# kan-bayashi/espnet

Measured on AMD Instinct MI355X. Metric: frames/sec, 12L Conformer hybrid CTC/attention training step (B=32 T=1000 d=256 per GPU), higher is better.
Workload: dtype f32; 1 GPU; BASELINE configs[1]: 12L Conformer enc d=256 h=4 ff=2048 k=31 macaron+cnn rel_pos, 6L Transformer dec, V=5000, fbank B=32 T=1000 L=100, mtlalpha 0.3, lsm 0.1; global_batch=32, frames=1000, parallelism=dp1, optimizer=adam+noam, clip 5.0, launch=hipGraph, wgrad_side_stream=False, optimizer_steps_done=113

## Files before the change

espnet_amd/csrc/gemm.hip:

```cpp
#include <stdlib.h>
#include "common.h"
#include "../../include/espnet_amd.h"

namespace {

constexpr int BK = 32;
constexpr int NTHREADS = 256;

template <int BM, int BN, int PREC>
struct Smem {
  static constexpr int LDK = PREC ? 40 : 36;
  using elem_t = typename std::conditional<PREC == 1, unsigned short, float>::type;
  elem_t a[2][BM][LDK];
  elem_t b[2][BN][LDK];
  int poff[3][BK];
};

struct RowState {
  int base;
  int ih, jw;
  int ok;
};

__device__ __forceinline__ RowState decompose(const eamd_gather_t& g, int row, int nrows) {
  RowState s;
  s.ok = row < nrows;
  int r = s.ok ? row : 0;
  int j = r % g.Wo;
  int t = r / g.Wo;
  int i = t % g.Ho;
  int b = t / g.Ho;
  s.base = b * g.Hin * g.Win;
  s.ih = i * g.sh;
  s.jw = j * g.sw;
  return s;
}

__device__ __forceinline__ long gather_off(const eamd_gather_t& g, const RowState& s, int tap) {
  int hh = s.ih + g.dh[tap];
  int ww = s.jw + g.dw[tap];
  bool ok = s.ok && hh >= 0 && hh < g.Hin && ww >= 0 && ww < g.Win;
  return ok ? ((long)(s.base + hh * g.Win + ww)) * g.C : -1L;
}

__device__ __forceinline__ float4 apply_act4(float4 v, int act) {
  if (act == EAMD_ACT_SWISH) {
    v.x = eamd_swish(v.x); v.y = eamd_swish(v.y); v.z = eamd_swish(v.z); v.w = eamd_swish(v.w);
  } else if (act == EAMD_ACT_RELU) {
    v.x = fmaxf(v.x, 0.f); v.y = fmaxf(v.y, 0.f); v.z = fmaxf(v.z, 0.f); v.w = fmaxf(v.w, 0.f);
  }
  return v;
}

__device__ __forceinline__ float4 load_kcontig(const float* __restrict__ rowp, bool row_ok, int k, int K,
                                               bool vec_ok) {
  float4 v = make_float4(0.f, 0.f, 0.f, 0.f);
  if (row_ok) {
    if (vec_ok && k + 3 < K) {
      v = *reinterpret_cast<const float4*>(rowp + k);
    } else {
      if (k + 0 < K) v.x = rowp[k + 0];
      if (k + 1 < K) v.y = rowp[k + 1];
      if (k + 2 < K) v.z = rowp[k + 2];
      if (k + 3 < K) v.w = rowp[k + 3];
    }
  }
  return v;
}

__device__ __forceinline__ float4 load_kstrided(const float* __restrict__ p, long ld, bool col_ok, int k,
                                                int K) {
  float4 v = make_float4(0.f, 0.f, 0.f, 0.f);
  if (col_ok) {
    const float* q = p + (long)k * ld;
    if (k + 3 < K) {
      v.x = q[0]; v.y = q[ld]; v.z = q[2 * ld]; v.w = q[3 * ld];
    } else {
      if (k + 0 < K) v.x = q[0];
      if (k + 1 < K) v.y = q[ld];
      if (k + 2 < K) v.z = q[2 * ld];
      if (k + 3 < K) v.w = q[3 * ld];
    }
  }
// ... 301 lines not shown
      if (p.precision == 0 && tile == 128 && t128 > 256 && t128 < 400 && p.splitk == 1) tile = 64;
    }
  }
  if (tile != 64 && tile != 128) return EAMD_EINVAL;

  if (p.gather.enabled) {
    const eamd_gather_t& g = p.gather;
    if (g.ntap < 1 || g.ntap > 9 || g.C <= 0 || g.C % BK != 0) return EAMD_EINVAL;
    if (!p.transA) {
      if (p.K != g.ntap * g.C) return EAMD_EINVAL;
    } else {
      if (p.M != g.ntap * g.C) return EAMD_EINVAL;
      if (g.C % tile != 0) return EAMD_EINVAL;
    }
  }
  if ((p.N + tile - 1) / tile > 65535) return EAMD_EUNSUPPORTED;
  if (p.h_dtype != 0 && p.h_dtype != 1) return EAMD_EINVAL;
  if (p.in_dtype == 1 && p.h_dtype != 0) return EAMD_EUNSUPPORTED;
  if (p.in_dtype != 1 && ((p.Hb && !(p.h_dtype == 1 && p.precision == 0)) || (p.drop_p != 0.f && p.precision != 0)))
    return EAMD_EUNSUPPORTED;
  if ((p.a_drop_p != 0.f || p.b_drop_p != 0.f) && (p.in_dtype != 0 || p.precision != 0)) return EAMD_EUNSUPPORTED;
  tile_out = tile;
  return EAMD_OK;
}

extern "C" int eamd_gemm(const eamd_gemm_t* pp, void* stream_) {
  if (!pp) return EAMD_EINVAL;
  eamd_gemm_t p = *pp;
  hipStream_t stream = (hipStream_t)stream_;
  int tile = 0;
  const int chk = gemm_check(p, tile);
  if (chk != EAMD_OK) return chk;
  const bool stats = p.epilogue == 7, rowgrad = p.epilogue == 8;
  if (p.in_dtype == 1) return eamd_gemm_bf16_dispatch(p, tile, stream);

  if (p.precision == 1 && p.gather.enabled && p.transA && !p.Hb && p.drop_p == 0.f && p.a_drop_p == 0.f &&
      p.b_drop_p == 0.f) {
    const int rc = eamd_gemm_f32_dispatch(p, tile, stream);
    if (rc != EAMD_EUNSUPPORTED) return rc;
  }
  if (p.precision == 0) {
    const int rc = eamd_gemm_f32_dispatch(p, tile, stream);
    if (rc != EAMD_EUNSUPPORTED) return rc;
    if (p.drop_p != 0.f || p.a_drop_p != 0.f || p.b_drop_p != 0.f || p.Hb) return EAMD_EUNSUPPORTED;
  }
  if (stats || rowgrad) return EAMD_EUNSUPPORTED;
  if (tile == 128) {
    return p.precision ? launch<128, 128, 1>(p, stream) : launch<128, 128, 0>(p, stream);
  }
  return p.precision ? launch<64, 64, 1>(p, stream) : launch<64, 64, 0>(p, stream);
}

int eamd_gemm_f32_multi(const eamd_gemm_t* ps, const int* tiles, int n, hipStream_t stream);

extern "C" int eamd_gemm_multi(const eamd_gemm_t* descs, int n, void* stream) {
  if (!descs || n < 1) return EAMD_EINVAL;
  if (n >= 2 && n <= EAMD_GEMM_MULTI_MAX) {
    eamd_gemm_t ps[EAMD_GEMM_MULTI_MAX];
    int tiles[EAMD_GEMM_MULTI_MAX];
    bool f32 = true;
    for (int i = 0; i < n; ++i) {
      ps[i] = descs[i];
      const int chk = gemm_check(ps[i], tiles[i]);
      if (chk != EAMD_OK) return chk;
      f32 = f32 && ps[i].in_dtype == 0 && ps[i].precision == 0;
    }
    if (f32) {
      const int rc = eamd_gemm_f32_multi(ps, tiles, n, (hipStream_t)stream);
      if (rc != EAMD_EUNSUPPORTED) return rc;
    }
  }
  for (int i = 0; i < n; ++i) {
    const int rc = eamd_gemm(&descs[i], stream);
    if (rc != EAMD_OK) return rc;
  }
  return EAMD_OK;
}

int eamd_gemm_f32_group_count(const eamd_gemm_t& p);
int eamd_gemm_f32_group_launch(const eamd_gemm_t* tab, const int* first, int n, int total, int tile, hipStream_t s);
int eamd_gemm_bf16_group_count(const eamd_gemm_t& p);
int eamd_gemm_bf16_group_launch(const eamd_gemm_t* tab, const int* first, int n, int total, int tile, hipStream_t s);

extern "C" int eamd_gemm_group_plan(const eamd_gemm_t* descs, int n, int32_t* first) {
  if (!descs || !first || n <= 0) return EAMD_EINVAL;
  long total = 0;
  for (int i = 0; i < n; ++i) {
    const eamd_gemm_t& p = descs[i];
    if (!p.A || !p.B || !p.C || p.M <= 0 || p.N <= 0 || p.K <= 0) return EAMD_EINVAL;
    if (p.in_dtype != descs[0].in_dtype || p.precision != descs[0].precision) return EAMD_EINVAL;
    if ((p.tile == 128) != (descs[0].tile == 128)) return EAMD_EINVAL;
    const int c = p.in_dtype == 1 ? eamd_gemm_bf16_group_count(p) : eamd_gemm_f32_group_count(p);
    if (c < 0) return c;
    first[i] = (int32_t)total;
    total += c;
    if (total >= (1L << 30)) return EAMD_EUNSUPPORTED;
  }
  first[n] = (int32_t)total;
  return (int)total;
}

extern "C" int eamd_gemm_group_launch(const eamd_gemm_t* descs_dev, const int32_t* first_dev, int n, int total, int in_dtype,
                                      int tile, void* stream) {
  if (!descs_dev || !first_dev || n <= 0 || total <= 0 || (tile != 64 && tile != 128)) return EAMD_EINVAL;
  return in_dtype == 1 ? eamd_gemm_bf16_group_launch(descs_dev, first_dev, n, total, tile, (hipStream_t)stream)
                       : eamd_gemm_f32_group_launch(descs_dev, first_dev, n, total, tile, (hipStream_t)stream);
}

extern "C" int eamd_abi_version(void) { return 1; }
```

espnet_amd/csrc/gemm_bf16.hip:

```cpp
#include <stdlib.h>
#include <type_traits>
#include "common.h"
#include "../../include/espnet_amd.h"

#include "gemm_bf16_common.h"

namespace {

template <int BM, int BN, bool TA, bool TB, bool FAST, bool GAT, bool ACT, bool ROWEPI = false>
__device__ __forceinline__ void gemm_bf16_body(const eamd_gemm_t& p, const int bid, const int nblk, const int zb) {
  constexpr int WM = BM / 2, WN = BN / 2;
  constexpr int MT = WM / 16, NTL = WN / 16;
  constexpr int NCA = BM / 32, NCB = BN / 32;
  constexpr int CPR_A = BM / 8, RPP_A = NT_ / CPR_A;
  constexpr int CPR_B = BN / 8, RPP_B = NT_ / CPR_B;
  using S = SmemB<BM, BN, TA, TB>;
  extern __shared__ __attribute__((aligned(16))) char smem_raw[];
  S& sm = *reinterpret_cast<S*>(smem_raw);

  const int t = threadIdx.x;
  const int lane = t & 63, wave = t >> 6;
  const int wm = wave >> 1, wn = wave & 1;
  const int tiles_n = (p.N + BN - 1) / BN;
  int tile_id, split;
  if (nblk < 0) {
    const int ntile = ((p.M + BM - 1) / BM) * tiles_n;
    const int per = (-nblk) >> 3;
    const int v = (bid & 7) * per + (bid >> 3);
    if (v >= ntile * p.splitk) return;
    split = v / ntile;
    tile_id = v - split * ntile;
  } else if (p.splitk > 1) {
    split = bid % p.splitk;
    tile_id = bid / p.splitk;
  } else {
    split = 0;
    const int ntile = nblk;
    const int id = bid, q = ntile >> 3, r = ntile & 7, xcd = id & 7, j = id >> 3;
    tile_id = (xcd < r ? xcd * (q + 1) : r * (q + 1) + (xcd - r) * q) + j;
  }
  const int tile_m = tile_id / tiles_n, tile_n = tile_id % tiles_n;
  const int m0 = tile_m * BM, n0 = tile_n * BN;
  const int b1 = zb / p.batch2, b2 = zb % p.batch2;
  const bf16_t* __restrict__ A = reinterpret_cast<const bf16_t*>(p.A) + b1 * p.sA1 + b2 * p.sA2;
  const bf16_t* __restrict__ B = reinterpret_cast<const bf16_t*>(p.B) + b1 * p.sB1 + b2 * p.sB2;
  const long coff = b1 * p.sC1 + b2 * p.sC2;

  const int nkt_total = (p.K + BK - 1) / BK;
  const int per = (nkt_total + p.splitk - 1) / p.splitk;
  const int kt_begin = split * per;
  const int kt_end = min(nkt_total, kt_begin + per);
  const int nkt = kt_end - kt_begin;

  constexpr bool gat = GAT;
  const bool a_vec = (p.lda % 8 == 0) && ((reinterpret_cast<uintptr_t>(A) & 15) == 0);
  const bool b_vec = (p.ldb % 8 == 0) && ((reinterpret_cast<uintptr_t>(B) & 15) == 0);

  int a_r[NCA], a_c[NCA], b_r[NCB], b_c[NCB];
#pragma unroll
  for (int i = 0; i < NCA; ++i) {
    if constexpr (TA) { a_r[i] = t / CPR_A + RPP_A * i; a_c[i] = t % CPR_A; }
    else              { a_r[i] = t / 8 + 32 * i;        a_c[i] = t % 8; }
  }
#pragma unroll
  for (int i = 0; i < NCB; ++i) {
    if constexpr (TB) { b_r[i] = t / CPR_B + RPP_B * i; b_c[i] = t % CPR_B; }
    else              { b_r[i] = t / 8 + 32 * i;        b_c[i] = t % 8; }
  }
  long a_off[NCA], b_off[NCB];
  if constexpr (FAST && !gat) {
#pragma unroll
    for (int i = 0; i < NCA; ++i) {
      if constexpr (!TA) a_off[i] = (long)min(m0 + a_r[i], p.M - 1) * p.lda + a_c[i] * 8;
      else a_off[i] = (long)a_r[i] * p.lda + min(m0 + a_c[i] * 8, (p.M - 1) & ~7);
    }
  }
  if constexpr (FAST) {
#pragma unroll
    for (int i = 0; i < NCB; ++i) {
      if constexpr (!TB) b_off[i] = (long)min(n0 + b_r[i], p.N - 1) * p.ldb + b_c[i] * 8;
      else b_off[i] = (long)b_r[i] * p.ldb + min(n0 + b_c[i] * 8, (p.N - 1) & ~7);
    }
  }
  RowStateB a_rs[NCA];
  if constexpr (gat && !TA) {
#pragma unroll
    for (int i = 0; i < NCA; ++i) a_rs[i] = decompose_b(p.gather, m0 + a_r[i], p.M);
  }
  GatherRegs gr = {0ull, 0ull, 1, 0, 0};
  if constexpr (gat) gr = gather_regs(p.gather);
  constexpr int DEPTH = BM >= 128 ? 3 : 4;
  constexpr int UNROLL = DEPTH % 2 ? 2 * DEPTH : DEPTH;
  uint4 ra[DEPTH][NCA], rb[DEPTH][NCB];
  const bool do_colsum = TA && p.colsum != nullptr && !gat && tile_n == 0;
  float cs[8];
#pragma unroll
  for (int j = 0; j < 8; ++j) cs[j] = 0.f;

  auto fill_poff = [&](int kt, int slot) __attribute__((always_inline)) {
    if (t < BK) {
      const int tap = m0 / gr.C;
      RowStateB s = decompose_b(p.gather, kt * BK + t, p.K);
      sm.poff[slot][t] = (int)gather_off_r(gr, s, tap);
    }
  };

  auto load_tile = [&](auto set_c, auto guard_c, int kt) __attribute__((always_inline)) {
    constexpr int SET = decltype(set_c)::value;
    constexpr bool GUARD = decltype(guard_c)::value;
    const int k0 = kt * BK;
    if constexpr (!TA) {
      if constexpr (!gat) {
#pragma unroll
        for (int i = 0; i < NCA; ++i) {
          const int m = m0 + a_r[i], k = k0 + a_c[i] * 8;
          if constexpr (FAST) {
            const int kk = (GUARD && k >= p.K) ? -a_c[i] * 8 : k0;
            ra[SET][i] = *reinterpret_cast<const uint4*>(A + a_off[i] + kk);
          } else {
            const int nv = m < p.M ? min(8, p.K - k) : 0;
            ra[SET][i] = load8(A, (long)m * p.lda + k, nv, a_vec);
          }
        }
      } else {
        const int tap = k0 / gr.C, c0 = k0 - tap * gr.C;
#pragma unroll
        for (int i = 0; i < NCA; ++i) {
          const long off = gather_off_r(gr, a_rs[i], tap);
          ra[SET][i] = load8_fast(A, off + c0 + a_c[i] * 8, off >= 0 ? 8 : 0);
        }
      }
    } else {
      if constexpr (!gat) {
#pragma unroll
// ... 416 lines not shown
```

espnet_amd/csrc/gemm_f32.hip:

```cpp
#include <stdlib.h>
#include <type_traits>
#include "common.h"
#include "../../include/espnet_amd.h"

#include "gemm_bf16_common.h"

namespace {

constexpr int FBK = 32;

template <int BM, int BN, bool TA, bool TB>
struct SmemF {
  static constexpr int KPAD_A = BM >= 128 ? 8 : 4, KPAD_B = BN >= 128 ? 8 : 4;
  static constexpr int LDA = TA ? BM + KPAD_A : FBK + 4;
  static constexpr int RA = TA ? FBK : BM;
  static constexpr int LDB = TB ? BN + KPAD_B : FBK + 4;
  static constexpr int RB = TB ? FBK : BN;
  static constexpr int OPS = 2 * (RA * LDA + RB * LDB);
  static constexpr int CT = BM * (BN + 4);
  float ab[OPS > CT ? OPS : CT];
  int poff[8][FBK];
  __device__ float* a(int buf) { return ab + buf * RA * LDA; }
  __device__ float* b(int buf) { return ab + 2 * RA * LDA + buf * RB * LDB; }
};

__device__ __forceinline__ float4 act4(float4 v, int act) {
  if (act == EAMD_ACT_SWISH) return make_float4(eamd_swish(v.x), eamd_swish(v.y), eamd_swish(v.z), eamd_swish(v.w));
  return make_float4(fmaxf(v.x, 0.f), fmaxf(v.y, 0.f), fmaxf(v.z, 0.f), fmaxf(v.w, 0.f));
}
__device__ __forceinline__ float4 mask4(float4 v, int nv) {
  return make_float4(nv > 0 ? v.x : 0.f, nv > 1 ? v.y : 0.f, nv > 2 ? v.z : 0.f, nv > 3 ? v.w : 0.f);
}

template <int BM, int BN, bool TA, bool TB, bool GAT, bool ACT, bool ROWEPI = false, bool NOPAD = false>
__device__ __forceinline__ void gemm_f32_body(const eamd_gemm_t& p, const int bid, const int nblk, const int zb) {
  constexpr int WM = BM / 2, WN = BN / 2;
  constexpr int MT = WM / 16, NTL = WN / 16;
  constexpr int NCA = BM / 32, NCB = BN / 32;
  constexpr int CPR_A = BM / 4, RPP_A = NT_ / CPR_A;
  constexpr int CPR_B = BN / 4, RPP_B = NT_ / CPR_B;
  using S = SmemF<BM, BN, TA, TB>;
  extern __shared__ __attribute__((aligned(16))) char smem_raw[];
  S& sm = *reinterpret_cast<S*>(smem_raw);

  const int t = threadIdx.x;
  const int lane = t & 63, wave = t >> 6;
  const int wm = wave >> 1, wn = wave & 1;
  const int tiles_n = (p.N + BN - 1) / BN;
  int tile_id, split;
  if (nblk < 0) {
    const int ntile = ((p.M + BM - 1) / BM) * tiles_n;
    const int per = (-nblk) >> 3;
    const int v = (bid & 7) * per + (bid >> 3);
    if (v >= ntile * p.splitk) return;
    split = v / ntile;
    tile_id = v - split * ntile;
  } else if (p.splitk > 1) {
    split = bid % p.splitk;
    tile_id = bid / p.splitk;
  } else {
    split = 0;
    const int ntile = nblk;
    const int id = bid, q = ntile >> 3, r = ntile & 7, xcd = id & 7, j = id >> 3;
    tile_id = (xcd < r ? xcd * (q + 1) : r * (q + 1) + (xcd - r) * q) + j;
  }
  const int tile_m = tile_id / tiles_n, tile_n = tile_id % tiles_n;
  const int m0 = tile_m * BM, n0 = tile_n * BN;
  const int b1 = zb / p.batch2, b2 = zb % p.batch2;
  const float* __restrict__ A = p.A + b1 * p.sA1 + b2 * p.sA2;
  const float* __restrict__ B = p.B + b1 * p.sB1 + b2 * p.sB2;
  const long coff = b1 * p.sC1 + b2 * p.sC2;

  const int nkt_total = (p.K + FBK - 1) / FBK;
  const int per = (nkt_total + p.splitk - 1) / p.splitk;
  const int kt_begin = split * per;
  const int kt_end = min(nkt_total, kt_begin + per);
  const int nkt = kt_end - kt_begin;

  int a_r[NCA], a_c[NCA], b_r[NCB], b_c[NCB];
#pragma unroll
  for (int i = 0; i < NCA; ++i) {
    if constexpr (TA) { a_r[i] = t / CPR_A + RPP_A * i; a_c[i] = t % CPR_A; }
    else              { a_r[i] = t / 8 + 32 * i;        a_c[i] = t % 8; }
  }
#pragma unroll
  for (int i = 0; i < NCB; ++i) {
    if constexpr (TB) { b_r[i] = t / CPR_B + RPP_B * i; b_c[i] = t % CPR_B; }
    else              { b_r[i] = t / 8 + 32 * i;        b_c[i] = t % 8; }
  }
  long a_off[NCA], b_off[NCB];
  if constexpr (!GAT) {
#pragma unroll
    for (int i = 0; i < NCA; ++i) {
      if constexpr (!TA) a_off[i] = (long)min(m0 + a_r[i], p.M - 1) * p.lda + a_c[i] * 4;
      else a_off[i] = (long)a_r[i] * p.lda + min(m0 + a_c[i] * 4, (p.M - 1) & ~3);
    }
  }
#pragma unroll
  for (int i = 0; i < NCB; ++i) {
    if constexpr (!TB) b_off[i] = (long)min(n0 + b_r[i], p.N - 1) * p.ldb + b_c[i] * 4;
    else b_off[i] = (long)b_r[i] * p.ldb + min(n0 + b_c[i] * 4, (p.N - 1) & ~3);
  }
  RowStateB a_rs[NCA];
  unsigned long long dh_pack = 0ull, dw_pack = 0ull;
  int gC = 1, gHin = 0, gWin = 0;
  if constexpr (GAT) {
#pragma unroll
    for (int tp = 0; tp < 9; ++tp) {
      dh_pack |= (unsigned long long)((unsigned)(p.gather.dh[tp] + 8) & 15u) << (4 * tp);
      dw_pack |= (unsigned long long)((unsigned)(p.gather.dw[tp] + 8) & 15u) << (4 * tp);
    }
    gC = p.gather.C; gHin = p.gather.Hin; gWin = p.gather.Win;
  }
  const int pK = p.K;
  const long ldaL = p.lda, ldbL = p.ldb;
  auto tap_dh = [&](int tap) __attribute__((always_inline)) { return (int)((dh_pack >> (4 * tap)) & 15ull) - 8; };
  auto tap_dw = [&](int tap) __attribute__((always_inline)) { return (int)((dw_pack >> (4 * tap)) & 15ull) - 8; };
  auto goff = [&](const RowStateB& rs, int dh, int dw) __attribute__((always_inline)) -> long {
    const int hh = rs.ih + dh, ww = rs.jw + dw;
    const bool ok = rs.ok && hh >= 0 && hh < gHin && ww >= 0 && ww < gWin;
    return ok ? ((long)(rs.base + hh * gWin + ww)) * gC : -1L;
  };
  constexpr bool g_nopad = NOPAD;
  if constexpr (GAT && !TA) {
#pragma unroll
    for (int i = 0; i < NCA; ++i) a_rs[i] = decompose_b(p.gather, m0 + a_r[i], p.M);
  }
  int pr_row = 0, pr_j = 0, pr_i = 0, pr_b = 0;
  if constexpr (GAT && TA) {
    if (t < FBK) {
      pr_row = kt_begin * FBK + t;
      pr_j = pr_row % p.gather.Wo;
      const int tt = pr_row / p.gather.Wo;
      pr_i = tt % p.gather.Ho;
      pr_b = tt / p.gather.Ho;
    }
  }
  constexpr int DEPTH = BM >= 128 ? 2 : 3;
  constexpr int UNROLL = DEPTH % 2 ? 2 * DEPTH : DEPTH;
  float4 ra[DEPTH][NCA], rb[DEPTH][NCB];
  const unsigned a_dseed = (ACT && p.a_drop_p > 0.f) ? eamd_drop_seed((const unsigned long long*)p.drop_step, p.a_drop_salt) : 0u;
  const unsigned b_dseed = (ACT && p.b_drop_p > 0.f) ? eamd_drop_seed((const unsigned long long*)p.drop_step, p.b_drop_salt) : 0u;
  const bool do_colsum = TA && p.colsum != nullptr && !GAT && tile_n == 0;
  float cs[4] = {0.f, 0.f, 0.f, 0.f};

  const int gWo = GAT ? p.gather.Wo : 1, gHo = GAT ? p.gather.Ho : 1, gsh = GAT ? p.gather.sh : 0, gsw = GAT ? p.gather.sw : 0;
  const int ta_tap = (GAT && TA) ? m0 / gC : 0;
  const int ta_dh = tap_dh(ta_tap), ta_dw = tap_dw(ta_tap);
  auto fill_poff = [&](int kt, int slot) __attribute__((always_inline)) {
    if (t < FBK) {
      RowStateB s;
      s.ok = pr_row < pK;
      s.base = pr_b * gHin * gWin; s.ih = pr_i * gsh; s.jw = pr_j * gsw;
      sm.poff[slot][t] = (int)goff(s, ta_dh, ta_dw);
      pr_row += FBK; pr_j += FBK;
      while (pr_j >= gWo) { pr_j -= gWo; ++pr_i; }
      while (pr_i >= gHo) { pr_i -= gHo; ++pr_b; }
    }
  };
// ... 523 lines not shown
```

espnet_amd/ops.py:

```python
import ctypes as C
import os
import math

import torch

from . import _lib
from ._lib import GatherT, GemmT, RowMapT, check, ptr, stream_ptr

ACT_NONE, ACT_RELU, ACT_SWISH = 0, 1, 2
EPI_NONE, EPI_RELU, EPI_SWISH, EPI_MUL_RELU_MASK, EPI_MUL_DSWISH, EPI_MUL_AUX, EPI_DACT_FACTOR, EPI_ROW_STATS, EPI_ROW_GRAD = 0, 1, 2, 3, 4, 5, 6, 7, 8

_PRECISIONS = {"fp32": 0, "bf16": 1}
_state = {"precision": 0}


def set_precision(name):
    if name not in _PRECISIONS:
        raise ValueError(f"precision must be one of {list(_PRECISIONS)}")
    _state["precision"] = _PRECISIONS[name]


def get_precision():
    return [k for k, v in _PRECISIONS.items() if v == _state["precision"]][0]

# ... 95 lines not shown
        assert (Cm is None and Cb is None) if epilogue == EPI_ROW_STATS else Cm is not None
    c32 = Cm if (Cm is not None and Cm.dtype == torch.float32) else None
    c16 = Cb if Cb is not None else (Cm if (Cm is not None and Cm.dtype == torch.bfloat16) else None)
    if c16 is not None and (c16.dtype != torch.bfloat16 or not bf):
        raise _lib.EamdError("gemm: bf16 outputs need bf16 operands")
    for tt in (R, bias, colsum):
        if tt is not None and tt.dtype != torch.float32:
            raise _lib.EamdError("gemm: bias / residual / colsum must be float32")
    b1, b2 = batch
    if gather is None:
        a_span = _span(K, lda, M) if transA else _span(M, lda, K)
        a_need = a_off + (b1 - 1) * sA[0] + (b2 - 1) * sA[1] + a_span
        if a_need > A.numel():
            raise _lib.EamdError(f"gemm: A too small ({A.numel()} < {a_need})")
    b_span = _span(K, ldb, N) if transB else _span(N, ldb, K)
    b_need = b_off + (b1 - 1) * sB[0] + (b2 - 1) * sB[1] + b_span
    if b_need > B.numel():
        raise _lib.EamdError(f"gemm: B too small ({B.numel()} < {b_need})")
    if cmap is None:
        c_need = c_off + (b1 - 1) * sC[0] + (b2 - 1) * sC[1] + _span(M, ldc, N)
        for ct in (c32, c16):
            if ct is not None and c_need > ct.numel():
                raise _lib.EamdError(f"gemm: C too small ({ct.numel()} < {c_need})")
    if bias is not None and bias.numel() < N:
        raise _lib.EamdError("gemm: bias too small")

    p = GemmT()
    p.A, p.B = ptr(A, a_off), ptr(B, b_off)
    p.C = ptr(c32, c_off) if c32 is not None else None
    p.Cb = ptr(c16, c_off) if c16 is not None else None
    p.bias = ptr(bias)
    p.aux = ptr(aux, c_off) if aux is not None else None
    p.aux_dtype = 1 if (aux is not None and aux.dtype == torch.bfloat16) else 0
    p.R = ptr(R, c_off) if R is not None else None
    if colsum is not None:
        if not transA or gather is not None or colsum.numel() < M * b1 * b2:
            raise _lib.EamdError("gemm: colsum needs transA, no gather and M outputs")
        p.colsum = ptr(colsum)
    p.M, p.N, p.K = M, N, K
    p.transA, p.transB = int(transA), int(transB)
    p.lda, p.ldb, p.ldc, p.ldaux, p.ldr = lda, ldb, ldc, ldaux or ldc, ldr or ldc
    p.batch1, p.batch2 = b1, b2
    p.sA1, p.sA2 = sA
    p.sB1, p.sB2 = sB
    p.sC1, p.sC2 = sC
    p.alpha, p.beta = alpha, beta
    p.a_act, p.b_act, p.epilogue = a_act, b_act, epilogue
    p.splitk = splitk
    p.in_dtype = 1 if bf else 0
    p.precision = 1 if bf else (_state["precision"] if precision is None else precision)
    p.tile = tile
    if stats is not None and epilogue == EPI_ROW_GRAD:
        rowc, col, fix, gscale, scale = stats
        if rowc.dtype != torch.float32 or rowc.numel() < 3 * M or col.dtype != torch.int32 or col.numel() < M or not (0 <= fix < N):
            raise _lib.EamdError("gemm: row-gradient coefficients too small or of the wrong dtype")
        p.stats.rowc, p.stats.col, p.stats.fix, p.stats.gscale, p.stats.scale = ptr(rowc), ptr(col), int(fix), ptr(gscale), float(scale)
    elif stats is not None:
        part, col, zcol, zfix, fix = stats
        tn = (N + tile - 1) // tile
        if part.dtype != torch.float32 or part.numel() < M * tn * 2 or zfix.numel() < M or not (0 <= fix < N) or \
                (col is not None and (col.dtype != torch.int32 or col.numel() < M or zcol is None or zcol.numel() < M)):
            raise _lib.EamdError("gemm: row-statistics buffers too small or of the wrong dtype")
        p.stats.part, p.stats.col, p.stats.zcol, p.stats.zfix, p.stats.fix = ptr(part), ptr(col), ptr(zcol), ptr(zfix), int(fix)
    if gather is not None:
        p.gather = gather
    if cmap is not None:
        p.cmap = cmap
    if drop is not None and drop[0] > 0.0:
        if ldc != N or c_off != 0 or (not bf and p.precision != 0):
            raise _lib.EamdError("gemm: fused dropout needs a contiguous [M, N] result and bf16 or fp32-MFMA operands")
        p.drop_p, p.drop_salt = float(drop[0]), int(drop[1])
        p.drop_step = ptr(rng_state(A.device))
        if Hb is not None:
            if Hb.dtype != (torch.bfloat16 if bf else torch.float32) or Hb.numel() < M * N:
                raise _lib.EamdError("gemm: Hb must be an [M, N] buffer of the operand dtype")
            p.Hb, p.h_act, p.h_dtype = ptr(Hb), h_act, 0 if bf else 1
    for which, d, ld_, off_, cols in (("a", a_drop, lda, a_off, (M if transA else K)), ("b", b_drop, ldb, b_off, (N if transB else K))):
        if d is not None and d[0] > 0.0:
            if bf or p.precision != 0 or ld_ != cols or off_ != 0 or b1 * b2 != 1 or gather is not None:
                raise _lib.EamdError("gemm: operand dropout needs an fp32-MFMA launch on a dense, unbatched operand")
            setattr(p, which + "_drop_p", float(d[0]))
            setattr(p, which + "_drop_salt", int(d[1]))
            p.drop_step = ptr(rng_state(A.device))
    if group and _wgroup["on"] and _in_grad_arena(Cm) and _wgroup_accepts(p):
        lo = Cm.data_ptr() + 4 * c_off
        hi = lo + 4 * _span(M, ldc, N)
        nbytes = A.numel() * A.element_size() + B.numel() * B.element_size()
        clash = any(lo < qhi and qlo < hi and (splitk == 1 or qsk == 1) for qlo, qhi, qsk in _wgroup["ranges"])
        if clash or _wgroup["bytes"] + nbytes > GROUP_WGRAD_MAX_BYTES:
            wgrad_group_flush()
        _wgroup["items"].append((p, (A, B, Cm, colsum)))
        _wgroup["ranges"].append((lo, hi, splitk))
        _wgroup["bytes"] += nbytes
        return
    if defer is not None:
        defer.append((p, (A, B, Cm, bias, aux, R, colsum, Cb, Hb, stats)))
        return
    if _gemm_record is not None:
        _gemm_record.append((p, (A, B, Cm, bias, aux, R, colsum, Cb, Hb, stats),
                             lambda sp, p=p: check(_lib.lib().eamd_gemm(C.byref(p), sp), "eamd_gemm")))
    check(_lib.lib().eamd_gemm(C.byref(p), stream_ptr()), "eamd_gemm")


GEMM_MULTI_MAX = 4


def gemm_multi(items):
    L = _lib.lib()
    for i0 in range(0, len(items), GEMM_MULTI_MAX):
        part = items[i0:i0 + GEMM_MULTI_MAX]
        arr = (GemmT * len(part))(*[it[0] for it in part])
        n = len(part)
        if _gemm_record is not None and any(it[0].in_dtype != 0 or it[0].precision != 0 for it in part):
            for p_, keep in part:
                _gemm_record.append((p_, keep, lambda sp, p_=p_: check(L.eamd_gemm(C.byref(p_), sp), "eamd_gemm")))
        elif _gemm_record is not None:
            _gemm_record.append((dict(kind="multi%d" % n, flop=sum(2.0 * it[0].M * it[0].N * it[0].K for it in part)),
                                 (arr, [it[1] for it in part]),
                                 lambda sp, arr=arr, n=n: check(L.eamd_gemm_multi(arr, n, sp), "eamd_gemm_multi")))
        check(L.eamd_gemm_multi(arr, n, stream_ptr()), "eamd_gemm_multi")


GROUP_WGRAD = True
STACK_WGRAD_MAX_ROWS = 64
GROUP_WGRAD_MAX_TILES = 384
GROUP_WGRAD_SK_DIV = 2
GROUP_WGRAD_TILE128_MIN = 100
GROUP_WGRAD_T128_WGS = 96
GROUP_WGRAD_MAX_BYTES = 16 << 30
_wgroup = {"on": False, "items": [], "ranges": [], "bytes": 0, "stack": {}, "pinned": [], "reserve": [], "arenas": {}}


def register_grad_arena(t):
    import weakref
    key = t.untyped_storage().data_ptr()
    _wgroup["arenas"][key] = weakref.ref(t)


def _in_grad_arena(t):
    key = t.untyped_storage().data_ptr()
    ref = _wgroup["arenas"].get(key)
    if ref is None:
        return False
    a = ref()
    if a is None or a.untyped_storage().data_ptr() != key:
        del _wgroup["arenas"][key]
        return False
    return True


def wgrad_group_begin():
    _wgroup["on"] = GROUP_WGRAD
    _wgroup["items"], _wgroup["stack"] = [], {}
    _wgroup["ranges"], _wgroup["bytes"] = [], 0


def _wgroup_accepts(p):
    if ((p.M + 63) // 64) * ((p.N + 63) // 64) > GROUP_WGRAD_MAX_TILES:
        return False
    first = (C.c_int32 * 2)()
    return _lib.lib().eamd_gemm_group_plan(C.byref(p), 1, first) > 0


def _wgroup_staging(nbytes):
    if torch.cuda.is_current_stream_capturing():
        for i, h in enumerate(_wgroup["reserve"]):
            if h.numel() >= nbytes:
                _wgroup["pinned"].append(_wgroup["reserve"].pop(i))
                return _wgroup["pinned"][-1][:nbytes]
        return None
    want = (nbytes + 4095) // 4096 * 4096 * 2
    _wgroup["reserve"] = [h for h in _wgroup["reserve"] if h.numel() >= want]
    while len(_wgroup["reserve"]) < 16:
        _wgroup["reserve"].append(torch.empty(want, dtype=torch.uint8, pin_memory=True))
    return torch.empty(nbytes, dtype=torch.uint8, pin_memory=True)


def wgrad_group_flush():
    stack, _wgroup["stack"] = _wgroup["stack"], {}
    for dW, db, dys, xs in stack.values():
        if len(dys) == 1:
            dyc, xc = dys[0], xs[0]
        else:
            dyc, xc = torch.cat(dys, 0), torch.cat(xs, 0)
        if dyc.shape[0] <= STACK_WGRAD_MAX_ROWS:
            sk = auto_splitk(dyc.shape[1], xc.shape[1], dyc.shape[0])
            gemm(dyc, xc, dW, dyc.shape[1], xc.shape[1], dyc.shape[0], dyc.shape[1], xc.shape[1], xc.shape[1], transA=1,
                 transB=1, splitk=sk, beta=1.0 if sk == 1 else 0.0, colsum=db, group=True)
        else:
            _linear_bwd_w(dyc, xc, dW, db=db)
    items = _wgroup["items"]
    if not items:
        return
    _wgroup["items"], _wgroup["ranges"], _wgroup["bytes"] = [], [], 0
    for tile in (64, 128):
        part = [it for it in items if (128 if it[0].tile == 128 else 64) == tile]
        if part:
            _wgroup_launch(part, tile)


def _wgroup_launch(items, tile):
    L = _lib.lib()

    def separately():
        for p, keep in items:
            if _gemm_record is not None:
                _gemm_record.append((p, keep, lambda sp, p=p: check(L.eamd_gemm(C.byref(p), sp), "eamd_gemm")))
            check(L.eamd_gemm(C.byref(p), stream_ptr()), "eamd_gemm")

    if len(items) == 1:
        return separately()
    n = len(items)
    dev = items[0][1][0].device
    arr = (GemmT * n)(*[it[0] for it in items])
    first = (C.c_int32 * (n + 1))()
    total = L.eamd_gemm_group_plan(arr, n, first)
    check(min(total, 0), "eamd_gemm_group_plan")
    nb_desc, nb_first = C.sizeof(arr), C.sizeof(first)
    host = _wgroup_staging(nb_desc + nb_first)
    if host is None:
        return separately()
    C.memmove(host.data_ptr(), arr, nb_desc)
    C.memmove(host.data_ptr() + nb_desc, first, nb_first)
    tab = torch.empty(nb_desc + nb_first, dtype=torch.uint8, device=dev)
    tab.copy_(host, non_blocking=True)
    in_dtype = int(arr[0].in_dtype)
    args = (ptr(tab), ptr(tab, nb_desc), n, total, in_dtype, tile)
    check(L.eamd_gemm_group_launch(*args, stream_ptr()), "eamd_gemm_group_launch")
    if _gemm_record is not None:
        _gemm_record.append((dict(kind="group%d" % tile, flop=sum(2.0 * it[0].M * it[0].N * it[0].K * it[0].batch1 * it[0].batch2 for it in items)),
                             (tab, [it[1] for it in items]),
                             lambda sp, args=args: check(L.eamd_gemm_group_launch(*args, sp), "eamd_gemm_group_launch")))


def cast_bf16(x, out=None):
    if out is None:
        out = torch.empty(x.shape, device=x.device, dtype=torch.bfloat16)
    assert x.dtype == torch.float32 and x.is_contiguous() and out.numel() == x.numel()
    check(_lib.lib().eamd_cast_bf16(ptr(x), ptr(out), C.c_int64(x.numel()), stream_ptr()), "eamd_cast_bf16")
    return out


def auto_splitk(m_out, n_out, k_red):
    tiles = ((m_out + 63) // 64) * ((n_out + 63) // 64)
    if tiles >= 512:
        return 1
    want = 4.0 * (128.0 / tiles) ** 0.5
    s = 1
    while s < want:
        s *= 2
    return max(1, min(s, 64, max(1, k_red // 128)))


LINEAR_ROWS = True
_infer = 0


class inference:

    def __enter__(self):
        global _infer
        _infer += 1

    def __exit__(self, *exc):
        global _infer
        _infer -= 1
        return False


def inference_call(fn):
    import functools

    @functools.wraps(fn)
    def wrapped(*a, **k):
        with inference():
            return fn(*a, **k)
    return wrapped
LINEAR_ROWS_MAX = 16
LINEAR_ROWS_BLOCK_MAX = 1024
LINEAR_ROWS_KSPLIT = True


def linear_fwd(x, W, b, out=None, *, act=EPI_NONE, R=None, alpha=1.0, a_act=ACT_NONE, out_dtype=torch.float32,
               drop=None, Hb=None, h_act=ACT_NONE, a_drop=None):
    M, K = x.shape
    N = W.shape[0]
    assert W.shape[1] == K and W.is_contiguous() and x.stride(1) == 1 and (R is None or R.stride(-1) == 1)
    if (LINEAR_ROWS and (M <= LINEAR_ROWS_MAX or (M <= LINEAR_ROWS_BLOCK_MAX and (K <= 512 or (K >= 1024 and LINEAR_ROWS_KSPLIT)) and N <= 1024
# ... 314 lines not shown
    if out is None:
        out = torch.empty(M, N, device=dev, dtype=torch.float32)
    p = _lib.RowProjT()
    p.a, p.lda, p.w, p.bias = ptr(a), a.stride(0), ptr(img), ptr(bias)
    p.R, p.ldr = ptr(R), (R.stride(0) if R is not None else 0)
    p.out, p.ldo = ptr(out), out.stride(0)
    p.M, p.K, p.N, p.alpha = M, K, N, float(alpha)
    if drop is not None and drop[0] > 0.0:
        p.p_out, p.salt_out, p.drop_step = float(drop[0]), int(drop[1]), ptr(rng_state(dev))
    if ln is not None:
        xr, g, b, eps, mean, rstd = ln
        p.ln_x, p.ln_w, p.ln_b, p.ln_mean, p.ln_rstd, p.ln_eps = ptr(xr), ptr(g), ptr(b), ptr(mean), ptr(rstd), float(eps)
    if affine is not None:
        sc, sh, act, a_out = affine
        p.a_scale, p.a_shift, p.a_act, p.a_out = ptr(sc), ptr(sh), int(act), ptr(a_out)
    if lnb is not None:
        xb, g, mean, rstd, dres, ws, d_out, d_ps = lnb
        p.lnb_x, p.lnb_gamma, p.lnb_mean, p.lnb_rstd, p.lnb_dres, p.lnb_ws = ptr(xb), ptr(g), ptr(mean), ptr(rstd), ptr(dres), ptr(ws)
        if d_out is not None:
            p.lnb_drop_out, p.lnb_drop_p, p.lnb_drop_salt, p.drop_step = ptr(d_out), float(d_ps[0]), int(d_ps[1]), ptr(rng_state(dev))
    fn = _lib.lib().eamd_rowproj
    keep = (a, img, bias, R, out, ln, affine, lnb)
    if _gemm_record is not None:
        _gemm_record.append((dict(kind="rowproj", flop=2.0 * M * K * N), keep, lambda sp, p=p: check(fn(C.byref(p), sp), "eamd_rowproj")))
    check(fn(C.byref(p), stream_ptr()), "eamd_rowproj")
    return out


def rowproj_lnb_ws(M, device):
    return torch.empty(int(_lib.lib().eamd_rowproj_lnb_workspace(M)), device=device, dtype=torch.float32)


_wgrad = {"stream": None, "used": False}


def enable_wgrad_stream(enable=True):
    _wgrad["stream"] = torch.cuda.Stream() if enable else None
    _wgrad["used"] = False


def wgrad_group_end():
    wgrad_group_flush()
    _wgroup["on"] = False


def wgrad_join():
    wgrad_group_flush()
    st = _wgrad["stream"]
    if st is not None and _wgrad["used"]:
        torch.cuda.current_stream().wait_stream(st)
        _wgrad["used"] = False


def linear_bwd_w(dy, x, dW, *, alpha=1.0, b_act=ACT_NONE, db=None, a_drop=None, b_drop=None, group=True):
    st = _wgrad["stream"]
    if st is None:
        return _linear_bwd_w(dy, x, dW, alpha=alpha, b_act=b_act, db=db, a_drop=a_drop, b_drop=b_drop, group=group)
    cur = torch.cuda.current_stream()
    st.wait_stream(cur)
    with torch.cuda.stream(st):
        _linear_bwd_w(dy, x, dW, alpha=alpha, b_act=b_act, db=db, a_drop=a_drop, b_drop=b_drop)
    dy.record_stream(st)
    x.record_stream(st)
    _wgrad["used"] = True


def _linear_bwd_w(dy, x, dW, *, alpha=1.0, b_act=ACT_NONE, db=None, a_drop=None, b_drop=None, group=True):
    M, N = dy.shape
    K = x.shape[1]
    assert x.shape[0] == M and dW.numel() == N * K and dW.dtype == torch.float32
    grouping = group and _wgroup["on"] and _wgrad["stream"] is None
    if (grouping and M <= STACK_WGRAD_MAX_ROWS and alpha == 1.0 and b_act == ACT_NONE
            and a_drop is None and b_drop is None and dy.is_contiguous() and x.is_contiguous() and _in_grad_arena(dW)):
        key = (dW.data_ptr(), db.data_ptr() if db is not None else 0, dy.dtype, x.dtype, N, K)
        _wgroup["stack"].setdefault(key, (dW, db, [], []))
        ent = _wgroup["stack"][key]
        ent[2].append(dy)
        ent[3].append(x)
        return
    sk = auto_splitk(N, K, M)
    tile = 0
    t64 = ((N + 63) // 64) * ((K + 63) // 64)
    if grouping and t64 <= GROUP_WGRAD_MAX_TILES and _in_grad_arena(dW):
        if t64 >= GROUP_WGRAD_TILE128_MIN and N >= 128 and K >= 128 and dy.dtype == torch.float32 and _state["precision"] == 0:
            tile = 128
            sk = max(1, min(GROUP_WGRAD_T128_WGS // (((N + 127) // 128) * ((K + 127) // 128)), M // 256))
        else:
            tile = 64
            sk = max(1, sk // GROUP_WGRAD_SK_DIV)
    gemm(dy, x, dW, N, K, M, N, K, K, transA=1, transB=1, alpha=alpha, b_act=b_act, splitk=sk, tile=tile,
         beta=1.0 if sk == 1 else 0.0, colsum=db, a_drop=a_drop, b_drop=b_drop, group=grouping)


def colsum(x, out, scale=1.0, rows=None, D=None, ld=None):
    rows = x.shape[0] if rows is None else rows
    D = x.shape[1] if D is None else D
    ld = D if ld is None else ld
    assert out.numel() >= D
    check(_lib.lib().eamd_colsum(ptr(x), C.c_int64(ld), ptr(out), C.c_int64(rows), D, C.c_float(scale),
                                 1 if x.dtype == torch.bfloat16 else 0, stream_ptr()), "eamd_colsum")


def layernorm_fwd(x, gamma, beta, eps, out_dtype=torch.float32):
    rows, D = x.shape
    y = torch.empty(rows, D, device=x.device, dtype=out_dtype)
    mean = torch.empty(rows, device=x.device, dtype=torch.float32)
    rstd = torch.empty(rows, device=x.device, dtype=torch.float32)
    y32, y16 = (ptr(y), None) if out_dtype == torch.float32 else (None, ptr(y))
    check(_lib.lib().eamd_layernorm_fwd(ptr(x), ptr(gamma), ptr(beta), y32, y16, ptr(mean), ptr(rstd), rows, D,
                                        C.c_float(eps), stream_ptr()), "eamd_layernorm_fwd")
    return y, mean, rstd


class _LnReduceJob(C.Structure):
    _fields_ = [("ws", C.c_void_p), ("dgamma", C.c_void_p), ("dbeta", C.c_void_p), ("nblk", C.c_int32), ("D", C.c_int32)]


defer_ln_reduce = True
_ln_pending = []
_ln_task = -1


def flush_ln_reduce():
    global _ln_pending, _ln_task
    jobs, _ln_pending, _ln_task = _ln_pending, [], -1
    if not jobs:
        return
    tab = (_LnReduceJob * len(jobs))()
    for i, (ws, dg, db, nblk, D) in enumerate(jobs):
        tab[i].ws, tab[i].dgamma, tab[i].dbeta, tab[i].nblk, tab[i].D = ws.data_ptr(), dg.data_ptr(), db.data_ptr(), nblk, D
    with torch.cuda.device(jobs[0][0].device):
        check(_lib.lib().eamd_layernorm_bwd_reduce(tab, len(jobs), stream_ptr()), "eamd_layernorm_bwd_reduce")


def ln_partials_reduce(ws, dgamma, dbeta, nblk, D):
    if _defer_ln(ws, dgamma, dbeta, nblk, D):
        return
    tab = (_LnReduceJob * 1)()
    tab[0].ws, tab[0].dgamma, tab[0].dbeta, tab[0].nblk, tab[0].D = ws.data_ptr(), dgamma.data_ptr(), dbeta.data_ptr(), nblk, D
    check(_lib.lib().eamd_layernorm_bwd_reduce(tab, 1, stream_ptr()), "eamd_layernorm_bwd_reduce")


def _defer_ln(ws, dgamma, dbeta, nblk, D):
    global _ln_pending, _ln_task
    if not defer_ln_reduce or not (getattr(dgamma, "_eamd_arena", False) and getattr(dbeta, "_eamd_arena", False)):
        return False
    task = torch._C._current_graph_task_id()
    if task < 0:
        return False
    if task != _ln_task:
        _ln_pending = []
        torch.autograd.Variable._execution_engine.queue_callback(flush_ln_reduce)
        _ln_task = task
    _ln_pending.append((ws, dgamma, dbeta, nblk, D))
    return True


def layernorm_bwd(dy, x, gamma, mean, rstd, dres, dgamma, dbeta, drop=None):
    rows, D = x.shape
    assert dy.shape == x.shape and dgamma.numel() == D and dbeta.numel() == D
    dx = torch.empty_like(x)
    L = _lib.lib()
    nws = int(L.eamd_layernorm_bwd_workspace(rows, D))
    ws = torch.empty(nws, device=x.device, dtype=torch.float32)
    pg, pb = ptr(dgamma), ptr(dbeta)
    if _defer_ln(ws, dgamma, dbeta, nws // (2 * D), D):
        pg = pb = None
    if drop is not None:
        dx16 = torch.empty(rows, D, device=x.device, dtype=act_dtype())
        fn, name = ((L.eamd_layernorm_bwd_drop, "eamd_layernorm_bwd_drop") if fast()
                    else (L.eamd_layernorm_bwd_drop_f32, "eamd_layernorm_bwd_drop_f32"))
        check(fn(ptr(dy), ptr(x), ptr(gamma), ptr(mean), ptr(rstd), ptr(dres), ptr(dx), ptr(dx16),
# ... 1429 lines not shown
```

include/espnet_amd.h:

```cpp
#ifndef ESPNET_AMD_H_
#define ESPNET_AMD_H_
#include <stdint.h>
#ifdef __cplusplus
extern "C" {
#endif

int eamd_abi_version(void);

typedef struct {
  int32_t enabled;
  int32_t C;
  int32_t ntap;
  int32_t Ho, Wo;
  int32_t Hin, Win;
  int32_t sh, sw;
  int32_t dh[9], dw[9];
} eamd_gather_t;

typedef struct {
  int32_t enabled;
  int32_t Ho, Wo;
  int32_t Hc, Wc;
  int32_t sh, oh, sw, ow;
} eamd_rowmap_t;

typedef struct {
  const float* A; const float* B; float* C;
  const float* bias; const float* aux; const float* R;
  float* colsum;
  int32_t M, N, K;
  int32_t transA, transB;
  int64_t lda, ldb, ldc, ldaux, ldr;
  int32_t batch1, batch2;
  int64_t sA1, sA2, sB1, sB2, sC1, sC2;
  float alpha, beta;
  int32_t a_act, b_act, epilogue;
  int32_t splitk;
  int32_t precision;
  int32_t tile;
  eamd_gather_t gather;
  eamd_rowmap_t cmap;
  void* Cb;
  int32_t in_dtype;
  int32_t aux_dtype;
  float drop_p;
  uint64_t drop_salt;
  const uint64_t* drop_step;
  void* Hb;
  int32_t h_act;
  float a_drop_p, b_drop_p;
  uint64_t a_drop_salt, b_drop_salt;
  int32_t h_dtype;
  struct {
    float* part; const int32_t* col; float* zcol; float* zfix; int32_t fix; int32_t reserved;
    const float* rowc; const float* gscale; float scale; int32_t reserved2;
  } stats;
} eamd_gemm_t;

int eamd_gemm(const eamd_gemm_t* p, void* stream);

#define EAMD_GEMM_MULTI_MAX 4
int eamd_gemm_multi(const eamd_gemm_t* descs, int n, void* stream);

int eamd_gemm_group_plan(const eamd_gemm_t* descs, int n, int32_t* first);
int eamd_gemm_group_launch(const eamd_gemm_t* descs_dev, const int32_t* first_dev, int n, int total, int in_dtype, int tile,
                           void* stream);

typedef struct {
  const float* x; const float* w1; const float* b1; const float* w2; const float* b2; const float* R;
  float* out; float* f; float* h;
  int32_t M, D, F, act;
  float alpha;
  float p_in; uint64_t salt_in; float p_out; uint64_t salt_out; const void* drop_step;
  int32_t dtype;
  int32_t hsplit;
  const float* ln_x; const float* ln_w; const float* ln_b; float* ln_mean; float* ln_rstd;
  float ln_eps; int32_t reserved2;
  const float* lnb_x; const float* lnb_gamma; const float* lnb_mean; const float* lnb_rstd; const float* lnb_dres;
  float* lnb_ws; float* lnb_drop_out; uint64_t lnb_drop_salt; float lnb_drop_p; int32_t reserved3;
} eamd_ffn_t;
int eamd_ffn_fwd(const eamd_ffn_t* p, void* stream);
int eamd_ffn_bwd(const eamd_ffn_t* p, void* stream);
typedef struct {
  const float* w1; const float* w2;
  float* fwd_first; float* fwd_second; float* bwd_first; float* bwd_second;
  int32_t D, F;
} eamd_ffn_pack_t;
int eamd_ffn_pack_f32_multi(const eamd_ffn_pack_t* jobs, int njobs, void* stream);

typedef struct {
  const float* a; int64_t lda;
  const float* w; const float* bias;
  const float* R; int64_t ldr;
  float* out; int64_t ldo;
  int32_t M, K, N, a_act;
  float alpha; float p_out; uint64_t salt_out; const void* drop_step;
  const float* ln_x; const float* ln_w; const float* ln_b; float* ln_mean; float* ln_rstd; float ln_eps; float lnb_drop_p;
  const float* a_scale; const float* a_shift; float* a_out;
  const float* lnb_x; const float* lnb_gamma; const float* lnb_mean; const float* lnb_rstd; const float* lnb_dres;
  float* lnb_ws; float* lnb_drop_out; uint64_t lnb_drop_salt;
} eamd_rowproj_t;
typedef struct {
  const float* w; float* image;
  int32_t K, N, ldw, trans;
} eamd_rowproj_pack_t;
int eamd_rowproj(const eamd_rowproj_t* p, void* stream);
int eamd_rowproj_pack_f32(const eamd_rowproj_pack_t* jobs, int njobs, void* stream);
int64_t eamd_rowproj_lnb_workspace(int M);
int eamd_ffn_pack_f32(const float* w1, const float* w2, float* fwd_first, float* fwd_second, float* bwd_first, float* bwd_second,
                      int D, int F, void* stream);
int eamd_ffn_pack_bf16(const void* w1, const void* w2, void* fwd_first, void* fwd_second, void* bwd_first, void* bwd_second,
                       int D, int F, void* stream);

int eamd_layernorm_fwd(const float* x, const float* gamma, const float* beta, float* y, void* y_bf16, float* mean,
                       float* rstd, int rows, int D, float eps, void* stream);
int64_t eamd_layernorm_bwd_workspace(int rows, int D);
typedef struct {
  const float* ws; float* dgamma; float* dbeta;
  int32_t nblk, D;
} eamd_ln_reduce_job_t;
int eamd_layernorm_bwd_reduce(const eamd_ln_reduce_job_t* jobs, int njobs, void* stream);
int eamd_layernorm_bwd(const float* dy, const float* x, const float* gamma, const float* mean,
                       const float* rstd, const float* dres, float* dx, float* dgamma, float* dbeta,
                       float* workspace, int rows, int D, void* stream);
int eamd_layernorm_bwd_drop(const float* dy, const float* x, const float* gamma, const float* mean, const float* rstd,
                            const float* dres, float* dx, void* dx_drop_bf16, float drop_p, const uint64_t* step_dev,
                            uint64_t salt, float* dgamma, float* dbeta, float* workspace, int rows, int D, void* stream);
int eamd_layernorm_bwd_drop_f32(const float* dy, const float* x, const float* gamma, const float* mean, const float* rstd,
                                const float* dres, float* dx, float* dx_drop, float drop_p, const uint64_t* step_dev,
                                uint64_t salt, float* dgamma, float* dbeta, float* workspace, int rows, int D, void* stream);

int eamd_softmax_fwd(const float* ac, const float* bd, const unsigned char* mask, int64_t mask_bstride,
                     int64_t mask_qstride, float* P, void* P_bf16, int nblocks, int B, int T1, int T2, int64_t ld,
                     float scale, void* stream);
int eamd_softmax_bwd(const float* P, const void* P_bf16, float* dP, float* dbd, void* dS_bf16, void* dbd_bf16,
                     int nblocks, int T1, int T2, int64_t ld, float scale, void* stream);

int eamd_attn_fwd(const void* qu, int64_t ldq, const void* qv, int64_t ldqv, const void* k, int64_t ldk, const void* v,
                  int64_t ldv, const void* pos, int64_t ldpos, const unsigned char* mask, int64_t mask_bstride,
                  int64_t mask_qstride, void* P_bf16, int64_t ldp, void* ctx_bf16, int64_t ldc, int B, int H, int T1,
                  int T2, int dk, float scale, void* Pd_bf16, float drop_p, const uint64_t* drop_step, uint64_t drop_salt,
                  const int32_t* shift_len, void* stream);

int eamd_attn_bwd_q(const void* dctx, int64_t ldd, const void* k, int64_t ldk, const void* v, int64_t ldv,
                    const void* P_bf16, int64_t ldp, void* dS_bf16, void* dbd_bf16, void* dq, int64_t ldo, int dq_is_bf16,
                    int B, int H, int T1, int T2, int dk, float scale, float drop_p, const uint64_t* drop_step,
                    uint64_t drop_salt, const int32_t* shift_len, void* stream);
// ... 315 lines not shown
```

Baseline: 1.129 million frames/s.

## Plan split-K globally across grouped weight-gradient GEMMs and sort by slice length

The grouped wgrad planner now picks each GEMM's split-K factor from a global work budget (CU slots × rounds), sorts the GEMMs by longest K slice first, and pads each GEMM's work-group count to a multiple of 8. Python no longer picks per-GEMM split-K for grouped wgrads; it seeds splitk=2 (atomic accumulate, beta=1) for large reductions. The kernels now split the K tiles evenly instead of using ceil-sized chunks. The aim is to balance load and cut the tail in the grouped launch. The cost is more atomic accumulation traffic, and the plan function now rewrites the caller's descriptor array.

```diff
diff --git a/espnet_amd/csrc/gemm.hip b/espnet_amd/csrc/gemm.hip
--- a/espnet_amd/csrc/gemm.hip
+++ b/espnet_amd/csrc/gemm.hip
@@ -1,4 +1,6 @@
 #include <stdlib.h>
+#include <algorithm>
+#include <vector>
 #include "common.h"
 #include "../../include/espnet_amd.h"
 
@@ -466,20 +468,51 @@
 int eamd_gemm_bf16_group_count(const eamd_gemm_t& p);
 int eamd_gemm_bf16_group_launch(const eamd_gemm_t* tab, const int* first, int n, int total, int tile, hipStream_t s);
 
-extern "C" int eamd_gemm_group_plan(const eamd_gemm_t* descs, int n, int32_t* first) {
+constexpr int GROUP_CUS = 256;
+constexpr int GROUP_ROUNDS = 12;
+constexpr int GROUP_MIN_SLICE_ROWS = 256;
+
+extern "C" int eamd_gemm_group_plan(eamd_gemm_t* descs, int n, int32_t* first) {
   if (!descs || !first || n <= 0) return EAMD_EINVAL;
-  long total = 0;
+  const bool bf = descs[0].in_dtype == 1;
+  const int T = descs[0].tile == 128 ? 128 : 64;
+  const int bk = bf ? 64 : 32;
+  const long slots = (long)GROUP_CUS * (T == 128 ? (bf ? 1 : 2) : 3);
+  std::vector<long> tiles(n), nkt(n);
+  long units = 0;
   for (int i = 0; i < n; ++i) {
     const eamd_gemm_t& p = descs[i];
     if (!p.A || !p.B || !p.C || p.M <= 0 || p.N <= 0 || p.K <= 0) return EAMD_EINVAL;
     if (p.in_dtype != descs[0].in_dtype || p.precision != descs[0].precision) return EAMD_EINVAL;
-    if ((p.tile == 128) != (descs[0].tile == 128)) return EAMD_EINVAL;
-    const int c = p.in_dtype == 1 ? eamd_gemm_bf16_group_count(p) : eamd_gemm_f32_group_count(p);
+    if ((p.tile == 128) != (T == 128)) return EAMD_EINVAL;
+    const int c = bf ? eamd_gemm_bf16_group_count(p) : eamd_gemm_f32_group_count(p);
     if (c < 0) return c;
-    first[i] = (int32_t)total;
-    total += c;
+    tiles[i] = (long)((p.M + T - 1) / T) * ((p.N + T - 1) / T);
+    nkt[i] = (p.K + bk - 1) / bk;
+    if (p.splitk > nkt[i]) return EAMD_EUNSUPPORTED;
+    units += tiles[i] * nkt[i];
+  }
+  const long lk = std::max<long>((GROUP_MIN_SLICE_ROWS + bk - 1) / bk, (units + slots * GROUP_ROUNDS - 1) / (slots * GROUP_ROUNDS));
+  std::vector<long> sk(n);
+  for (int i = 0; i < n; ++i) {
+    sk[i] = std::min(nkt[i], std::max<long>((nkt[i] + lk / 2) / lk, descs[i].splitk));
+    if (sk[i] > 65535) return EAMD_EUNSUPPORTED;
+  }
+  std::vector<int> order(n);
+  for (int i = 0; i < n; ++i) order[i] = i;
+  auto slice = [&](int i) { return (nkt[i] + sk[i] - 1) / sk[i]; };
+  std::stable_sort(order.begin(), order.end(), [&](int a, int b) { return slice(a) > slice(b); });
+  std::vector<eamd_gemm_t> sorted(n);
+  long total = 0;
+  for (int j = 0; j < n; ++j) {
+    const int i = order[j];
+    sorted[j] = descs[i];
+    sorted[j].splitk = (int)sk[i];
+    first[j] = (int32_t)total;
+    total += (tiles[i] * sk[i] + 7) / 8 * 8;
     if (total >= (1L << 30)) return EAMD_EUNSUPPORTED;
   }
+  std::copy(sorted.begin(), sorted.end(), descs);
   first[n] = (int32_t)total;
   return (int)total;
 }
diff --git a/espnet_amd/csrc/gemm_bf16.hip b/espnet_amd/csrc/gemm_bf16.hip
--- a/espnet_amd/csrc/gemm_bf16.hip
+++ b/espnet_amd/csrc/gemm_bf16.hip
@@ -47,9 +47,8 @@
   const long coff = b1 * p.sC1 + b2 * p.sC2;
 
   const int nkt_total = (p.K + BK - 1) / BK;
-  const int per = (nkt_total + p.splitk - 1) / p.splitk;
-  const int kt_begin = split * per;
-  const int kt_end = min(nkt_total, kt_begin + per);
+  const int kt_begin = (int)((long)split * nkt_total / p.splitk);
+  const int kt_end = (int)((long)(split + 1) * nkt_total / p.splitk);
   const int nkt = kt_end - kt_begin;
 
   constexpr bool gat = GAT;
diff --git a/espnet_amd/csrc/gemm_f32.hip b/espnet_amd/csrc/gemm_f32.hip
--- a/espnet_amd/csrc/gemm_f32.hip
+++ b/espnet_amd/csrc/gemm_f32.hip
@@ -72,9 +72,8 @@
   const long coff = b1 * p.sC1 + b2 * p.sC2;
 
   const int nkt_total = (p.K + FBK - 1) / FBK;
-  const int per = (nkt_total + p.splitk - 1) / p.splitk;
-  const int kt_begin = split * per;
-  const int kt_end = min(nkt_total, kt_begin + per);
+  const int kt_begin = (int)((long)split * nkt_total / p.splitk);
+  const int kt_end = (int)((long)(split + 1) * nkt_total / p.splitk);
   const int nkt = kt_end - kt_begin;
 
   int a_r[NCA], a_c[NCA], b_r[NCB], b_c[NCB];
diff --git a/espnet_amd/ops.py b/espnet_amd/ops.py
--- a/espnet_amd/ops.py
+++ b/espnet_amd/ops.py
@@ -201,15 +201,19 @@
             setattr(p, which + "_drop_p", float(d[0]))
             setattr(p, which + "_drop_salt", int(d[1]))
             p.drop_step = ptr(rng_state(A.device))
-    if group and _wgroup["on"] and _in_grad_arena(Cm) and _wgroup_accepts(p):
+    q = None
+    if group and _wgroup["on"] and _in_grad_arena(Cm):
+        q = GemmT.from_buffer_copy(p)
+        q.splitk, q.beta = (2 if K >= GROUP_WGRAD_ATOMIC_MIN_ROWS else 1), 1.0
+    if q is not None and _wgroup_accepts(q):
         lo = Cm.data_ptr() + 4 * c_off
         hi = lo + 4 * _span(M, ldc, N)
         nbytes = A.numel() * A.element_size() + B.numel() * B.element_size()
-        clash = any(lo < qhi and qlo < hi and (splitk == 1 or qsk == 1) for qlo, qhi, qsk in _wgroup["ranges"])
+        clash = any(lo < qhi and qlo < hi and (q.splitk == 1 or qsk == 1) for qlo, qhi, qsk in _wgroup["ranges"])
         if clash or _wgroup["bytes"] + nbytes > GROUP_WGRAD_MAX_BYTES:
             wgrad_group_flush()
-        _wgroup["items"].append((p, (A, B, Cm, colsum)))
-        _wgroup["ranges"].append((lo, hi, splitk))
+        _wgroup["items"].append((q, (A, B, Cm, colsum), p))
+        _wgroup["ranges"].append((lo, hi, q.splitk))
         _wgroup["bytes"] += nbytes
         return
     if defer is not None:
@@ -243,9 +247,8 @@
 GROUP_WGRAD = True
 STACK_WGRAD_MAX_ROWS = 64
 GROUP_WGRAD_MAX_TILES = 384
-GROUP_WGRAD_SK_DIV = 2
 GROUP_WGRAD_TILE128_MIN = 100
-GROUP_WGRAD_T128_WGS = 96
+GROUP_WGRAD_ATOMIC_MIN_ROWS = 512
 GROUP_WGRAD_MAX_BYTES = 16 << 30
 _wgroup = {"on": False, "items": [], "ranges": [], "bytes": 0, "stack": {}, "pinned": [], "reserve": [], "arenas": {}}
 
@@ -278,7 +281,8 @@
     if ((p.M + 63) // 64) * ((p.N + 63) // 64) > GROUP_WGRAD_MAX_TILES:
         return False
     first = (C.c_int32 * 2)()
-    return _lib.lib().eamd_gemm_group_plan(C.byref(p), 1, first) > 0
+    one = GemmT.from_buffer_copy(p)
+    return _lib.lib().eamd_gemm_group_plan(C.byref(one), 1, first) > 0
 
 
 def _wgroup_staging(nbytes):
@@ -322,7 +326,7 @@
     L = _lib.lib()
 
     def separately():
-        for p, keep in items:
+        for _q, keep, p in items:
             if _gemm_record is not None:
                 _gemm_record.append((p, keep, lambda sp, p=p: check(L.eamd_gemm(C.byref(p), sp), "eamd_gemm")))
             check(L.eamd_gemm(C.byref(p), stream_ptr()), "eamd_gemm")
@@ -803,12 +807,8 @@
     tile = 0
     t64 = ((N + 63) // 64) * ((K + 63) // 64)
     if grouping and t64 <= GROUP_WGRAD_MAX_TILES and _in_grad_arena(dW):
-        if t64 >= GROUP_WGRAD_TILE128_MIN and N >= 128 and K >= 128 and dy.dtype == torch.float32 and _state["precision"] == 0:
-            tile = 128
-            sk = max(1, min(GROUP_WGRAD_T128_WGS // (((N + 127) // 128) * ((K + 127) // 128)), M // 256))
-        else:
-            tile = 64
-            sk = max(1, sk // GROUP_WGRAD_SK_DIV)
+        big = t64 >= GROUP_WGRAD_TILE128_MIN and N >= 128 and K >= 128 and dy.dtype == torch.float32 and _state["precision"] == 0
+        tile = 128 if big else 64
     gemm(dy, x, dW, N, K, M, N, K, K, transA=1, transB=1, alpha=alpha, b_act=b_act, splitk=sk, tile=tile,
          beta=1.0 if sk == 1 else 0.0, colsum=db, a_drop=a_drop, b_drop=b_drop, group=grouping)
 
diff --git a/include/espnet_amd.h b/include/espnet_amd.h
--- a/include/espnet_amd.h
+++ b/include/espnet_amd.h
@@ -62,7 +62,7 @@
 #define EAMD_GEMM_MULTI_MAX 4
 int eamd_gemm_multi(const eamd_gemm_t* descs, int n, void* stream);
 
-int eamd_gemm_group_plan(const eamd_gemm_t* descs, int n, int32_t* first);
+int eamd_gemm_group_plan(eamd_gemm_t* descs, int n, int32_t* first);
 int eamd_gemm_group_launch(const eamd_gemm_t* descs_dev, const int32_t* first_dev, int n, int total, int in_dtype, int tile,
                            void* stream);
 
```

Result: no change. 1.135 million frames/s, median of 6 (+0.5%).
